# KrisKennaway/ii-vision

Measured on AMD Instinct MI355X. Metric: DHGR frames transcoded/sec, higher is better.
Workload: dtype u16; 1 GPU; DHGR NTSC palette 560x192 S-iid synthetic clips, 750 frames each, 14336 independent clips per GPU, Movie.encode control flow (490 opcodes/frame, bank flip per 2 KiB); palette=NTSC, streams_per_gpu=14336, greedy_form=shared, resident_clip_frames=750, opcodes_per_frame=490, parallelism=1 GPU x 14336 independent streams, no collective

## Files before the change

### ii-vision_amd/csrc/iiv_greedy.hip

```cpp
#include "iiv_host.h"
#include <cstdio>
#include <cstdlib>
#include <mutex>
#include <type_traits>
#include "iiv_stream.h"
#include "iiv_wave.h"

namespace iiv {

#ifndef IIV_WAVE_OCC
#define IIV_WAVE_OCC 6
#endif
#ifndef IIV_STEP_PRIO
#define IIV_STEP_PRIO 1
#endif

#ifndef IIV_SHARED_W
#define IIV_SHARED_W 8
#endif
#ifndef IIV_TAKE_CHECK_PLAIN
#define IIV_TAKE_CHECK_PLAIN 1
#endif
#ifndef IIV_TAKE_CHECK_SHARED
#define IIV_TAKE_CHECK_SHARED 0
#endif
#ifndef IIV_SHARED_W_HGR
#define IIV_SHARED_W_HGR 16
#endif
struct WaveLds {
    uint32_t nz[256];
    uint32_t pdone[256];
    uint32_t mt[624 + 256];
};
struct WaveLdsBits {
    uint32_t nz[256];
    uint32_t pdone[256];
};
#ifndef IIV_SHARED_HGR_HALVES
#define IIV_SHARED_HGR_HALVES 2
#endif
template <int MODE> struct SharedCfg {
    static constexpr int kOffsets = MODE == kDHGR ? 2 : IIV_SHARED_HGR_HALVES;
    static constexpr int kHalfBytes = 2 << (SplitTraits<MODE>::kLeftCBits + SplitTraits<MODE>::kLeftRowBits);
    static constexpr int kL1Bytes = kOffsets * kHalfBytes;
    static constexpr int kPad = kL1Bytes;
    static constexpr int kW = MODE == kDHGR ? IIV_SHARED_W : IIV_SHARED_W_HGR;
    static constexpr bool kMtRegs = MODE == kHGR && kOffsets == 2;
    static constexpr int kWaveBytes = kMtRegs ? (int)sizeof(WaveLdsBits) : (int)sizeof(WaveLds);
    static constexpr int kLds = kPad + kW * kWaveBytes;
    static_assert(kLds <= 160 * 1024, "a workgroup's LDS");
};

__device__ static inline WaveLds *own_wave_lds()
{
    __shared__ WaveLds w;
    return &w;
}

template <int MODE, int W, bool FOUR = false>
__global__ __launch_bounds__(64 * W, W == 1 ? IIV_WAVE_OCC : MODE == kHGR ? (W + 3) / 4 : (2 * W + 3) / 4 + (W % 4 ? 1 : 0)) void greedy_wave_kernel(StreamState *__restrict__ states,
                                                                   const uint8_t *__restrict__ frames_main,
                                                                   const uint8_t *__restrict__ frames_aux, int n_frames,
                                                                   const LaunchSeg *__restrict__ segs, int seg_stride,
                                                                   const NarrowTables nt,
                                                                   uint8_t *__restrict__ ops_out, size_t ops_stride, int n_streams, int bank, int *__restrict__ queue,
                                                                   int count_stats, const int *__restrict__ perm, uint32_t *__restrict__ cost)
{
    using T = SplitTraits<MODE>;
    constexpr uint32_t INF = 0xffffffffu;
    typedef uint32_t __attribute__((aligned(2))) u32_a2;
    using SC = SharedCfg<MODE>;
    extern __shared__ uint32_t dyn_lds[];
    const int lane0 = W == 1 ? (int)threadIdx.x : (int)(threadIdx.x & 63);
    const int wave = W == 1 ? 0 : IIV_SGPR(threadIdx.x >> 6);
    constexpr bool kMtRegs = W > 1 && SC::kMtRegs;
    uint32_t *nz, *pdone, *mt;
    if constexpr (W == 1) {
        __shared__ uint32_t nz_s[256], pdone_s[256], mt_s[624 + 256];
        nz = nz_s, pdone = pdone_s, mt = mt_s;
    } else if constexpr (kMtRegs) {
        WaveLdsBits *wl = reinterpret_cast<WaveLdsBits *>(reinterpret_cast<char *>(dyn_lds) + SC::kPad) + wave;
        nz = wl->nz, pdone = wl->pdone, mt = nullptr;
    } else {
        WaveLds *wl = reinterpret_cast<WaveLds *>(reinterpret_cast<char *>(dyn_lds) + SC::kPad) + wave;
        nz = wl->nz, pdone = wl->pdone, mt = wl->mt;
    }
    const char *const l1_lds = reinterpret_cast<const char *>(dyn_lds);
    if (W > 1) {
        uint4 *dst = reinterpret_cast<uint4 *>(dyn_lds);
        constexpr int kQuads = SC::kHalfBytes / 16;
#pragma unroll
        for (int h = 0; h < SC::kOffsets; h++) {
            const int o = byte_offset<MODE>(h, bank);
            const uint4 *src = reinterpret_cast<const uint4 *>(nt.base + ((size_t)o << (T::kLeftCBits + T::kLeftRowBits + 1)));
            for (int i = threadIdx.x; i < kQuads; i += 64 * W) dst[h * kQuads + i] = src[i];
        }
        __syncthreads();
    }

    auto run_stream = [&](const int stream, const int lane) {
    const unsigned long long clk0 = __builtin_amdgcn_s_memtime();
    StreamState &S = states[stream];
    const LaunchSeg g = segs[(size_t)stream * seg_stride];
    const int n_ops = IIV_SGPR(g.n_ops), is_aux = IIV_SGPR(g.is_aux), frame = IIV_SGPR(g.frame);
    if (n_ops <= 0) return;
    if (W > 1 && is_aux != bank) {
        if (lane == 0 && !S.error) S.error = kErrBankMix;
        return;
    }
    uint8_t *out = ops_out + (size_t)stream * ops_stride + (size_t)IIV_SGPR(g.ops_base) * 6;

    if (!S.gen_active || S.error) {
        if (lane == 0 && !S.error) S.error = kErrNoGenerator;
        return;
    }
    for (int i = lane; i < 256; i += 64) {
        nz[i] = S.nzbits[i];
        pdone[i] = S.pdone[i];
    }
    if constexpr (!kMtRegs)
        for (int i = lane; i < 624; i += 64) mt[i] = S.mt_py[i];
    if (W == 1) __syncthreads(); else wave_lds_sync();
    uint32_t *ahead = mt + 624;
    auto gen_ahead = [&]() {
#pragma unroll
        for (int k = 0; k < 4; k++) {
            const int i = lane + 64 * k;
            if (k < 3 || i < 227) ahead[i] = mt[i + 397] ^ mt_mix(mt[i], mt[i + 1]);
        }
        wave_lds_sync();
        {
            const int i = 192 + lane;
            if (i >= 227) ahead[i] = ahead[i - 227] ^ mt_mix(mt[i], mt[i + 1]);
        }
        wave_lds_sync();
    };
    auto gen_rest = [&]() {
#pragma unroll
        for (int k = 0; k < 6; k++) {
            const int i = 256 + 64 * k + lane;
            if (k < 5 || i < 624) {
                const uint32_t nv = i < 483 ? ahead[i - 227] : mt[i - 227];
                const uint32_t nx = i == 623 ? ahead[0] : mt[i + 1];
                const uint32_t v = nv ^ mt_mix(mt[i], nx);
                wave_lds_sync();
                mt[i] = v;
            }
            wave_lds_sync();
        }
    };
    auto move_head = [&]() {
#pragma unroll
        for (int k = 0; k < 4; k++) mt[lane + 64 * k] = ahead[lane + 64 * k];
        wave_lds_sync();
    };
    int mt_idx = IIV_SGPR(S.mt_py_idx);
    MtRegs mtr;
    const MtLaneConsts mtk(lane);
    uint32_t q_key = 0;
    int q_idx = 0, n_pend = 0, mt_behind = 0;
    constexpr int kQueueTrash = 63, kQueueHigh = 56;
    if constexpr (kMtRegs) {
        mt_regs_load(mtr, S.mt_py, lane);
        if (mt_idx >= 624) {
            mt_regs_twist(mtr, mtk);
            mt_idx -= 624;
        }
    } else {
        gen_ahead();
        if (mt_idx >= 624) {
            move_head();
            gen_rest();
            gen_ahead();
            mt_idx -= 624;
        }
    }
    bool twist_pending = false;
    auto twist_now = [&]() {
        if constexpr (!kMtRegs) {
            if (__builtin_expect(twist_pending, 0)) {
                gen_rest();
                gen_ahead();
                twist_pending = false;
            }
        }
    };

    const int n_sorted = IIV_SGPR(S.n_sorted);
    const int truncated = IIV_SGPR(S.truncated);
    int head = IIV_SGPR(S.head), n_pushed = IIV_SGPR(S.n_pushed), exhausted = IIV_SGPR(S.exhausted);
    int done = 0, err = 0;
    uint32_t draws = 0;
    unsigned long long pad_ops = 0;
    const uint32_t pad_content = (uint32_t)IIV_SGPR(S.pad_content);

    const int o_e = byte_offset<MODE>(0, is_aux), o_d = byte_offset<MODE>(1, is_aux);
    const uint32_t l1_e = (uint32_t)o_e << (T::kLeftCBits + T::kLeftRowBits + 1), l1_d = (uint32_t)o_d << (T::kLeftCBits + T::kLeftRowBits + 1);
    const uint32_t r1_e = nt.right_off + ((uint32_t)o_e << (T::kRightCBits + T::kRightRowBits + 1));
    const uint32_t r1_d = nt.right_off + ((uint32_t)o_d << (T::kRightCBits + T::kRightRowBits + 1));
    const __amdgpu_buffer_rsrc_t rsrc_s = __builtin_amdgcn_make_buffer_rsrc((void *)&S, 0, (int)sizeof(StreamState), 0x00020000);
    const int up_off = (int)offsetof(StreamState, up16) + is_aux * 8192 * 2, mem_off = (int)offsetof(StreamState, mem) + is_aux * 8192;
    const __amdgpu_buffer_rsrc_t rsrc = __builtin_amdgcn_make_buffer_rsrc((void *)nt.base, 0, 0x7fffffff, 0x00020000);
    const uint8_t *tgt_frames = (MODE == kDHGR && is_aux ? frames_aux : frames_main) +
                                ((size_t)stream * n_frames + frame) * 8192;
    const uint4 *wd_rows = reinterpret_cast<const uint4 *>(S.wd);
    const int wsel = lane >> 3;
    const int sh0 = (4 * lane) & 31;
    const uint32_t y0 = 4u * (uint32_t)lane;
    constexpr uint32_t kKeyMul = (1u << kWdDwShift) | (1u << 8);
    const uint32_t ycst0 = y0 - kNarrowBias * kKeyMul;

    struct Loaded {
        uint32_t gl[4], gr[4], kb[4];
    };
    auto gather8 = [&](const uint4 &w, uint32_t c, Loaded &L) {
        const uint32_t sl_e = (W == 1 ? l1_e : 0u) + (split_content_left<MODE>(c, 0) << (T::kLeftRowBits + 1));
        constexpr bool kOddInLds = W > 1 && SC::kOffsets == 2;
        const uint32_t sl_d = (kOddInLds ? (uint32_t)SC::kHalfBytes : l1_d) + (split_content_left<MODE>(c, 1) << (T::kLeftRowBits + 1));
        const uint32_t sr_e = r1_e + (split_content_right<MODE>(c, 0) << (T::kRightRowBits + 1));
        const uint32_t sr_d = r1_d + (split_content_right<MODE>(c, 1) << (T::kRightRowBits + 1));
        const uint32_t wr[4] = {w.x, w.y, w.z, w.w};
        uint32_t ol[4], orr[4];
#pragma unroll
        for (int r = 0; r < 4; r++) {
            ol[r] = wd_off_left(wr[r]);
            orr[r] = wd_off_right(wr[r]);
        }
        if (W == 1) {
            L.gl[0] = (uint16_t)__builtin_amdgcn_raw_buffer_load_b16(rsrc, (int)ol[0], (int)sl_e, 0);
            L.gl[2] = (uint16_t)__builtin_amdgcn_raw_buffer_load_b16(rsrc, (int)ol[2], (int)sl_e, 0);
            L.gl[1] = (uint16_t)__builtin_amdgcn_raw_buffer_load_b16(rsrc, (int)ol[1], (int)sl_d, 0);
            L.gl[3] = (uint16_t)__builtin_amdgcn_raw_buffer_load_b16(rsrc, (int)ol[3], (int)sl_d, 0);
        } else {
            L.gl[0] = *reinterpret_cast<const uint16_t *>(l1_lds + (sl_e + ol[0]));
            L.gl[2] = *reinterpret_cast<const uint16_t *>(l1_lds + (sl_e + ol[2]));
            if (kOddInLds) {
                L.gl[1] = *reinterpret_cast<const uint16_t *>(l1_lds + (sl_d + ol[1]));
                L.gl[3] = *reinterpret_cast<const uint16_t *>(l1_lds + (sl_d + ol[3]));
            } else {
                L.gl[1] = (uint16_t)__builtin_amdgcn_raw_buffer_load_b16(rsrc, (int)ol[1], (int)sl_d, 0);
                L.gl[3] = (uint16_t)__builtin_amdgcn_raw_buffer_load_b16(rsrc, (int)ol[3], (int)sl_d, 0);
            }
        }
        L.gr[0] = (uint16_t)__builtin_amdgcn_raw_buffer_load_b16(rsrc, (int)orr[0], (int)sr_e, 0);
        L.gr[2] = (uint16_t)__builtin_amdgcn_raw_buffer_load_b16(rsrc, (int)orr[2], (int)sr_e, 0);
        L.gr[1] = (uint16_t)__builtin_amdgcn_raw_buffer_load_b16(rsrc, (int)orr[1], (int)sr_d, 0);
        L.gr[3] = (uint16_t)__builtin_amdgcn_raw_buffer_load_b16(rsrc, (int)orr[3], (int)sr_d, 0);
#pragma unroll
        for (int r = 0; r < 4; r++) {
            L.kb[r] = (wr[r] << kWdDwShift) + (ycst0 + (uint32_t)r);
            asm volatile("" : "+v"(L.kb[r]));
        }
    };

    uint32_t ob0 = 0, ob1 = 0, ob2 = 0, ob3 = 0;
    int ob_base = 0, ob_n = 0;
    auto flush_ops = [&]() {
        if (lane < ob_n) {
            uint8_t *q = out + (size_t)(ob_base + lane) * 6;
            const uint32_t pg = (ob0 >> 8) & 31u, xx = ob0 & 255u, cc = (ob0 >> 16) & 255u;
            *reinterpret_cast<u32_a2 *>(q) = (pg + 32u) | (cc << 8) | (xx << 16) | (ob1 << 24);
            *reinterpret_cast<uint16_t *>(q + 4) = (uint16_t)((ob2 & 255u) | ((FOUR ? ob3 & 255u : xx) << 8));
        }
        ob_base = done;
        ob_n = 0;
    };

#ifdef IIV_STAMPS
    int n_ties = 0, n_tie_members = 0, n_ties_small = 0;
    int n_rel = 0, n_rel_single = 0, n_rel_double = 0;
#endif
    bool prev_tie = false;
    int n_exact = 0;
    uint32_t pkey_v = 0;
    int push_f1 = 0, push_f2 = 0, push_f3 = 0, push_base = 0;
    static_assert(kPushedCap >= 3 * 7680 + 8, "a generator's steps have distinct primaries: <= 7680 steps x <= 3 pushes");
    auto mt_resolve = [&](int a, int b, int off) -> uint32_t {
        const int lo = __builtin_amdgcn_readlane(q_idx, a) - off, hi = __builtin_amdgcn_readlane(q_idx, b - 1) - off;
        const bool in = lane >= a && lane < b;
        const uint32_t w = mt_regs_gather(mtr, in ? q_idx - off : lo, lo, hi);
        const uint32_t key = q_key | ((mt_temper(w) >> 24) << 13);
        const uint32_t slot = in ? (uint32_t)(n_pushed - n_pend + lane) * 4u : 0x7ffffff0u;
        __builtin_amdgcn_raw_buffer_store_b32(key, rsrc_s, (int)slot, (int)offsetof(StreamState, pushed), 0);
        return key;
    };
    auto mt_enqueue = [&](uint32_t keys, int k, int fk, int pos, int first) {
        const uint32_t key0 = (uint32_t)__builtin_amdgcn_readlane((int)keys, k);
        const int at = fk ? n_pend + pos : kQueueTrash;
        asm("s_mov_b32 m0, %4\n\tv_writelane_b32 %0, %2, m0\n\tv_writelane_b32 %1, %3, m0"
            : "+v"(q_key), "+v"(q_idx)
            : "s"(key0), "s"(first + pos), "s"(at));
    };
    auto mt_service = [&](int target) -> uint32_t {
        uint32_t keys = 0;
        for (;;) {
            const int r = (int)__popcll(__ballot(lane < n_pend && q_idx < 624));
            if (r > 0) {
                keys = mt_resolve(0, r, 0);
                if (r < n_pend) {
                    const int from = ((lane + r) & 63) << 2;
                    q_key = (uint32_t)__builtin_amdgcn_ds_bpermute(from, (int)q_key);
                    q_idx = __builtin_amdgcn_ds_bpermute(from, q_idx);
                }
                n_pend -= r;
            }
            if (mt_behind <= target) break;
            mt_regs_twist(mtr, mtk);
            mt_behind--;
            q_idx -= 624;
        }
        return keys;
    };
    auto apply = [&](auto track, uint32_t e, uint32_t W1, uint32_t W2, uint32_t W3, int C) {
        const int p = (e >> 8) & 31, x = e & 255;
        const uint32_t c = (e >> 16) & 0xffu;
        auto flag = [](uint32_t w) -> int {
            int f;
            asm("s_min_u32 %0, %1, 1" : "=s"(f) : "s"(w >> 8) : "scc");
            return f;
        };
        const int f1 = flag(W1), f2 = flag(W2), f3 = FOUR ? flag(W3) : 0;
        if (__builtin_expect(n_pushed > kPushedCap - 4, 0)) {
            err = kErrPushedOverflow;
            return;
        }
        if (__builtin_expect(twist_pending && mt_idx + C + (FOUR ? 3 : 2) >= 256, 0)) twist_now();
        uint32_t w_v = (uint32_t)x, k_v = 0u;
        asm("v_writelane_b32 %0, %2, 1\n\tv_writelane_b32 %0, %3, 2\n\tv_writelane_b32 %1, %4, 2"
            : "+v"(w_v), "+v"(k_v)
            : "s"(W1), "s"(W2), "s"(f1));
        if (FOUR)
            asm("v_writelane_b32 %0, %2, 3\n\tv_writelane_b32 %1, %3, 3" : "+v"(w_v), "+v"(k_v) : "s"(W3), "s"(f1 + f2));
        asm("s_mov_b32 m0, %4\n\tv_writelane_b32 %0, %3, m0\n\tv_writelane_b32 %1, %5, m0\n\tv_writelane_b32 %2, %6, m0"
            : "+v"(ob0), "+v"(ob1), "+v"(ob2)
            : "s"(IIV_SGPR(e)), "s"(ob_n), "s"(W1), "s"(W2));
        if (FOUR) asm("s_mov_b32 m0, %2\n\tv_writelane_b32 %0, %1, m0" : "+v"(ob3) : "s"(W3), "s"(ob_n));
        int ln = lane;
        asm volatile("" : "+v"(ln));
        uint32_t pk0_v = 0;
        if (ln < (FOUR ? 4 : 3)) {
            const uint32_t off = w_v & 255u, val = w_v >> 8;
            const uint32_t loc = (uint32_t)(p * 256) | off;
            __builtin_amdgcn_raw_buffer_store_b16((unsigned short)val, rsrc_s, (int)(loc * 2u), up_off, 0);
            __builtin_amdgcn_raw_buffer_store_b8((unsigned char)c, rsrc_s, (int)loc, mem_off, 0);
            const uint32_t gone_bit = (val == 0u ? 1u : 0u) << (off & 31u);
            atomicAnd(&nz[loc >> 5], ~gone_bit);
            atomicOr(&pdone[p * 8 + (x >> 5)], 1u << (x & 31));
            if constexpr (!kMtRegs) {
                const uint32_t nonce = mt_temper(mt[mt_idx + C + (int)k_v]) >> 24;
                const uint32_t pkey = ((2047u - val) << 21) | (nonce << 13) | loc;
                const uint32_t slot = val != 0u ? (uint32_t)(n_pushed + (int)k_v) * 4u : 0x7ffffff0u;
                __builtin_amdgcn_raw_buffer_store_b32(pkey, rsrc_s, (int)slot, (int)offsetof(StreamState, pushed), 0);
                if (decltype(track)::value) pkey_v = pkey;
            } else {
                pk0_v = ((2047u - val) << 21) | loc;
            }
        }
        if constexpr (kMtRegs) {
            const int first = mt_behind * 624 + mt_idx + C;
            mt_enqueue(pk0_v, 1, f1, 0, first);
            mt_enqueue(pk0_v, 2, f2, f1, first);
            if (FOUR) mt_enqueue(pk0_v, 3, f3, f1 + f2, first);
            n_pend += f1 + f2 + f3;
        }
        if (decltype(track)::value) push_f1 = f1, push_f2 = f2, push_f3 = f3, push_base = n_pushed;
        mt_idx += C + f1 + f2 + f3;
        draws += (uint32_t)(C + f1 + f2 + f3);
        n_pushed += f1 + f2 + f3;
        if constexpr (kMtRegs) {
            if (decltype(track)::value) {
                pkey_v = mt_service(0);
                if (n_pend > 0) {
                    const int r = (FOUR ? f1 + f2 + f3 : f1 + f2) - n_pend;
                    const uint32_t k2 = (uint32_t)__builtin_amdgcn_ds_bpermute(((lane - r) & 63) << 2, (int)mt_service(-1));
                    pkey_v = lane < r ? pkey_v : k2;
                }
            } else if (__builtin_expect(n_pend > kQueueHigh, 0)) {
                (void)mt_service(0);
            }
        }
        done++;
        ob_n++;
        if (__builtin_expect(ob_n == 64, 0)) flush_ops();
        if (__builtin_expect(mt_idx >= 624, 0)) {
            if constexpr (kMtRegs) {
                mt_idx -= 624;
                mt_behind++;
            } else {
                move_head();
                mt_idx -= 624;
                twist_pending = true;
            }
        }
    };

    auto step = [&](auto track, uint32_t e, const Loaded &L, uint32_t nzw, uint32_t pdw) -> bool {
        const int x = e & 255;
        const uint32_t c = (e >> 16) & 0xffu;
        const uint32_t xword = (uint32_t)__builtin_amdgcn_readlane((int)nzw, (x >> 5) * 8);
        if (__builtin_expect(!((xword >> (x & 31)) & 1u), 0)) return false;
        if (MODE == kDHGR && c >= 0x80) {
            err = kErrPaletteBit;
            return true;
        }
        const uint32_t xbit = wsel == (x >> 5) ? 1u << (x & 31) : 0u;
        nzw &= ~xbit;
        pdw |= xbit;
        uint32_t nd[4];
        int ke[4];
        int C = 0;
        unsigned long long cand[4];
#pragma unroll
        for (int r = 0; r < 4; r++) {
            nd[r] = L.gl[r] + L.gr[r];
            const int d = (int)(__umul24(nd[r], kKeyMul) + L.kb[r]);
            const int gone = __builtin_amdgcn_sbfe((int)pdw, sh0 + r, 1);
            const int live = __builtin_amdgcn_sbfe((int)nzw, sh0 + r, 1);
            ke[r] = d & live;
            cand[r] = __ballot((d & ~gone) < 0);
            C += (int)__popcll(cand[r]);
        }
        const int a0 = ke[0] < ke[1] ? ke[0] : ke[1], b0 = ke[0] < ke[1] ? ke[1] : ke[0];
        const int a1 = ke[2] < ke[3] ? ke[2] : ke[3], b1 = ke[2] < ke[3] ? ke[3] : ke[2];
        const int k1 = a0 < a1 ? a0 : a1, hi01 = a0 < a1 ? a1 : a0, mb = b0 < b1 ? b0 : b1;
        const int k2 = hi01 < mb ? hi01 : mb;
        const int k3 = hi01 < mb ? mb : hi01;
        auto nd_of = [&](int y) -> uint32_t {
            const uint32_t nd01 = nd[0] | (nd[1] << 16), nd23 = nd[2] | (nd[3] << 16);
            const uint32_t pa = (uint32_t)__builtin_amdgcn_readlane((int)nd01, y >> 2);
            const uint32_t pb = (uint32_t)__builtin_amdgcn_readlane((int)nd23, y >> 2);
            return ((((y & 2) ? pb : pa) >> ((y & 1) * 16)) & 0xffffu) - kNarrowBias;
        };
        uint32_t W1 = (uint32_t)x, W2 = (uint32_t)x, W3 = (uint32_t)x;
        bool tie = prev_tie;
        auto shared_delta = [&](int K) -> bool {
            uint32_t m = ((uint32_t)(ke[0] ^ K)) - 1u;
#pragma unroll
            for (int r = 1; r < 4; r++) {
                const uint32_t x1 = ((uint32_t)(ke[r] ^ K)) - 1u;
                m = x1 < m ? x1 : m;
            }
            return __ballot(m < (1u << kWdDwShift) - 1u) != 0ull;
        };
#ifdef IIV_STAMPS
        {
            int D1 = k1, D2 = k2;
            wave_top2_i32(D1, D2);
            if (D1 < 0 && D2 < 0 && ((D1 >> kWdDwShift) == (D2 >> kWdDwShift) || shared_delta(D2))) {
                int n1 = 0;
#pragma unroll
                for (int r = 0; r < 4; r++) n1 += (int)__popcll(__ballot(ke[r] < 0 && (ke[r] >> kWdDwShift) == (D1 >> kWdDwShift)));
                n_ties++;
                n_tie_members += n1;
                if (n1 <= 2) n_ties_small++;
                const int dR = n1 >= 2 ? (D1 >> kWdDwShift) : (D2 >> kWdDwShift);
                int lane_cnt = 0;
#pragma unroll
                for (int r = 0; r < 4; r++) lane_cnt += (ke[r] < 0 && (ke[r] >> kWdDwShift) == dR) ? 1 : 0;
                const unsigned long long b1 = __ballot(lane_cnt >= 1), b2 = __ballot(lane_cnt >= 2), b3 = __ballot(lane_cnt >= 3), b4 = __ballot(lane_cnt >= 4);
                n_rel += IIV_SGPR(__popcll(b1) + __popcll(b2) + __popcll(b3) + __popcll(b4));
                n_rel_single += IIV_SGPR(b2 == 0ull ? 1 : 0);
                n_rel_double += IIV_SGPR((b2 != 0ull && b3 == 0ull) ? 1 : 0);
            }
        }
#endif
        int K1 = k1, K2 = k2;
        if (!tie) wave_top2_i32(K1, K2); else K1 = K2 = 0;
        if (__builtin_expect(K1 < 0, 1)) {
            W1 = (uint32_t)K1 & 0x7ffffu;
            if (__builtin_expect(K2 < 0, 1)) {
                W2 = (uint32_t)K2 & 0x7ffffu;
                tie = (K1 >> kWdDwShift) == (K2 >> kWdDwShift);
                if constexpr (!FOUR) {
                    if (!tie) tie = shared_delta(K2);
                } else if (!tie) {
                    const int c3 = k1 > K2 ? k1 : (k2 > K2 ? k2 : k3);
                    const int K3 = wave_min_i32(c3);
                    if (K3 < 0) {
                        W3 = (uint32_t)K3 & 0x7ffffu;
                        tie = (K2 >> kWdDwShift) == (K3 >> kWdDwShift) || shared_delta(K3);
                    }
                }
            }
        }
        if (W > 1 ? __builtin_expect(tie, 0) : tie) {
            twist_now();
            n_exact++;
            static_assert(kWdDwShift == 20, "the key's delta field is taken from bits 20..31 of an eligible key");
            int key[4];
            int run = mt_idx;
#pragma unroll
            for (int q = 0; q < 4; q++) run += prefix_popc(cand[q]);
            uint32_t word[4];
            if constexpr (kMtRegs) {
                int at[4];
                bool mine[4];
#pragma unroll
                for (int r = 0; r < 4; r++) {
                    at[r] = run;
                    mine[r] = (cand[r] >> lane) & 1ull;
                    run += mine[r] ? 1 : 0;
                }
                const int last = mt_idx + (C > 0 ? C - 1 : 0), last0 = last < 623 ? last : 623;
                if (mt_behind != 0) (void)mt_service(0);
#pragma unroll
                for (int r = 0; r < 4; r++) word[r] = mt_regs_gather(mtr, mine[r] && at[r] < 624 ? at[r] : mt_idx, mt_idx, last0);
                if (__builtin_expect(last >= 624, 0)) {
                    (void)mt_service(-1);
#pragma unroll
                    for (int r = 0; r < 4; r++) {
                        const uint32_t w2 = mt_regs_gather(mtr, mine[r] && at[r] >= 624 ? at[r] - 624 : 0, 0, last - 624);
                        word[r] = at[r] >= 624 ? w2 : word[r];
                    }
                }
            } else {
#pragma unroll
                for (int r = 0; r < 4; r++) {
                    word[r] = mt[run];
                    run += (int)((cand[r] >> lane) & 1ull);
                }
            }
#pragma unroll
            for (int r = 0; r < 4; r++) {
                const uint32_t nonce = mt_temper(word[r]) >> 24;
                key[r] = (int)(((uint32_t)(ke[r] >> 4) & 0xffff0000u) | (nonce << 8) | (y0 + r));
            }
            const int ta0 = key[0] < key[1] ? key[0] : key[1], tb0 = key[0] < key[1] ? key[1] : key[0];
            const int ta1 = key[2] < key[3] ? key[2] : key[3], tb1 = key[2] < key[3] ? key[3] : key[2];
            const int t1 = ta0 < ta1 ? ta0 : ta1;
            const int thi = ta0 < ta1 ? ta1 : ta0, tmb = tb0 < tb1 ? tb0 : tb1;
            const int t2 = thi < tmb ? thi : tmb;
            int T1 = t1, T2 = t2;
            wave_top2_i32(T1, T2);
            W1 = T1 < 0 ? (nd_of(T1 & 255) << 8) | (uint32_t)(T1 & 255) : (uint32_t)x;
            W2 = T2 < 0 ? (nd_of(T2 & 255) << 8) | (uint32_t)(T2 & 255) : (uint32_t)x;
            prev_tie = T2 < 0 && (T1 >> 16) == (T2 >> 16);
            if constexpr (FOUR) {
                const int t3 = thi < tmb ? tmb : thi;
                const int T3 = wave_min_i32(t1 > T2 ? t1 : (t2 > T2 ? t2 : t3));
                W3 = T3 < 0 ? (nd_of(T3 & 255) << 8) | (uint32_t)(T3 & 255) : (uint32_t)x;
                prev_tie = prev_tie || (T3 < 0 && (T2 >> 16) == (T3 >> 16));
            }
        }
        apply(track, e, W1, W2, W3, C);
        return true;
    };

    int guard = n_ops + 8192 + 2 * kPushedCap + 64;
#ifdef IIV_STAMPS
    unsigned long long ph[4] = {0, 0, 0, 0}, ph_t = __builtin_amdgcn_s_memtime();
    const unsigned long long wave_t0 = ph_t, wave_r0 = __builtin_amdgcn_s_memrealtime();
    int n_steps = 0;
#define IIV_PHASE(i)                                                  \
    do {                                                              \
        const unsigned long long now_ = __builtin_amdgcn_s_memtime(); \
        ph[i] += now_ - ph_t;                                         \
        ph_t = now_;                                                  \
    } while (0)
#else
#define IIV_PHASE(i) do { } while (0)
#endif

    if (head < n_sorted && !exhausted) {
        int win_base = head, win_end = head;
        int n_dense = 0, qi = 0;
        uint32_t dense_e = 0;
        uint32_t ord_next = S.order[(head + lane) & 8191];
        auto refill = [&]() {
            const int start = win_end;
            const uint32_t e = ord_next;
            const int idx = start + lane;
            ord_next = S.order[(idx + 64) & 8191];
            const uint32_t loc = e & 0x1fffu;
            const bool v = idx < n_sorted && ((nz[loc >> 5] >> (loc & 31)) & 1u);
            const unsigned long long mask = __ballot(v);
            n_dense = (int)__popcll(mask);
            qi = 0;
            const int dst = v ? prefix_popc(mask) : n_dense + prefix_popc(~mask);
            dense_e = (uint32_t)__builtin_amdgcn_ds_permute(dst << 2, (int)((e & 0x00ffffffu) | ((uint32_t)lane << 24)));
            asm volatile("" : "+v"(dense_e));
            win_base = start;
            win_end = start + 64 < n_sorted ? start + 64 : n_sorted;
        };
        auto take = [&](int &next_head) -> uint32_t {
            for (;;) {
                while (__builtin_expect(qi >= n_dense, 0)) {
                    if (win_end >= n_sorted) return 0u;
                    refill();
                }
                const uint32_t e = (uint32_t)__builtin_amdgcn_readlane((int)dense_e, qi++);
                if constexpr ((W == 1 && IIV_TAKE_CHECK_PLAIN) || (W > 1 && IIV_TAKE_CHECK_SHARED)) {
                    const uint32_t loc = e & 0x1fffu;
                    const uint32_t w = IIV_SGPR(nz[loc >> 5]);
                    if (!((w >> (loc & 31)) & 1u)) continue;
                }
                next_head = win_base + (int)(e >> 24) + 1;
                return e | 0x80000000u;
            }
        };
        auto row_of = [&](uint32_t e) -> uint4 { return wd_rows[((e >> 8) & 31) * 64 + lane]; };

        uint32_t eA, eB, eC;
        int hA = head, hB, hC;
        uint4 rowP, rowQ;
        Loaded set0, set1;
        eA = take(hA);
        const uint4 rowA = row_of(eA);
        hB = hA;
        eB = eA ? take(hB) : 0u;
        rowP = row_of(eB);
        gather8(rowA, eA >> 16 & 0xffu, set0);
        hC = hB;
        eC = eB ? take(hC) : 0u;
        rowQ = row_of(eC);
        auto half = [&](const Loaded &cur, Loaded &nxt, uint4 &row, bool active) -> bool {
#ifdef IIV_STAMPS
            asm volatile("" : "+v"(row.x), "+v"(row.y), "+v"(row.z), "+v"(row.w));
            IIV_PHASE(3);
#endif
            const uint32_t nzA = nz[((eA >> 8) & 31) * 8 + wsel], pdA = pdone[((eA >> 8) & 31) * 8 + wsel];
            gather8(row, eB >> 16 & 0xffu, nxt);
            __builtin_amdgcn_sched_barrier(0);
            int hD = hC;
            const uint32_t eD = (active && eC) ? take(hD) : 0u;
            row = row_of(eD);
            IIV_PHASE(0);
            if (__builtin_expect(!active, 0)) return false;
            twist_now();
            IIV_PHASE(1);
#ifdef IIV_STAMPS
            n_steps++;
#endif
            __builtin_amdgcn_s_setprio(IIV_STEP_PRIO);
            (void)step(std::false_type{}, eA, cur, nzA, pdA);
            __builtin_amdgcn_s_setprio(0);
            IIV_PHASE(2);
            head = hA;
            eA = eB;
            hA = hB;
            eB = eC;
            hB = hC;
            eC = eD;
            hC = hD;
            if (__builtin_expect(--guard < 0, 0)) err = kErrGuard;
            return eA && done < n_ops && !err;
        };
        if (eA && done < n_ops) {
            bool more;
            do {
                more = half(set0, set1, rowP, true);
                more = half(set1, set0, rowQ, more);
            } while (more);
        }
        if (!eA && !err) head = n_sorted;
    }

    if (done < n_ops && !err && !exhausted) {
        if constexpr (kMtRegs) (void)mt_service(0);
        uint32_t ck = INF, ci = 0;
        for (int i = lane; i < n_pushed; i += 64) {
            const uint32_t k = S.pushed[i];
            ci = k < ck ? (uint32_t)i : ci;
            ck = k < ck ? k : ck;
        }
        auto writelane = [&](uint32_t &v, uint32_t val, int l) {
            asm("s_mov_b32 m0, %2\n\tv_writelane_b32 %0, %1, m0" : "+v"(v) : "s"(IIV_SGPR(val)), "s"(IIV_SGPR(l)));
        };
        auto wave_min_u32 = [&](uint32_t v) -> uint32_t { return (uint32_t)wave_min_i32((int)(v ^ 0x80000000u)) ^ 0x80000000u; };
        auto cache_merge = [&](uint32_t key, uint32_t idx) {
            const int sub = (int)(idx & 63u);
            const uint32_t cur = (uint32_t)__builtin_amdgcn_readlane((int)ck, sub);
            if (key < cur) {
                writelane(ck, key, sub);
                writelane(ci, idx, sub);
            }
        };
        while (done < n_ops && !err) {
            if (--guard < 0) {
                err = kErrGuard;
                break;
            }
            if (truncated) {
                err = kErrSortBudget;
                break;
            }
            const uint32_t bk = wave_min_u32(ck);
            if (bk == INF) {
                exhausted = 1;
                break;
            }
            const int wl = (int)__builtin_ctzll(__ballot(ck == bk));
            const uint32_t bi = (uint32_t)__builtin_amdgcn_readlane((int)ci, wl);
            if (lane == 0) S.pushed[bi] = INF;
            constexpr int kSub = (kPushedCap + 4095) / 4096;
            static_assert(kPushedCap <= 64 * 64 * kSub, "the rescan of a sub-bag must reach every index below kPushedCap");
            uint32_t rk[kSub], ridx[kSub];
#pragma unroll
            for (int t = 0; t < kSub; t++) {
                ridx[t] = (uint32_t)wl + 64u * (uint32_t)(lane + 64 * t);
                rk[t] = INF;
                if (ridx[t] < (uint32_t)n_pushed && ridx[t] != bi) rk[t] = S.pushed[ridx[t]];
            }
            const uint32_t loc = bk & 0x1fffu;
            const uint32_t c = (uint32_t)IIV_SGPR(tgt_frames[loc]);
            const uint32_t e = loc | (c << 16);
            const uint4 w = wd_rows[((e >> 8) & 31) * 64 + lane];
            Loaded L;
            gather8(w, c, L);
            twist_now();
            push_f1 = push_f2 = push_f3 = 0;
            (void)step(std::true_type{}, e, L, nz[((e >> 8) & 31) * 8 + wsel], pdone[((e >> 8) & 31) * 8 + wsel]);
            uint32_t mk = rk[0], mi = ridx[0];
#pragma unroll
            for (int t = 1; t < kSub; t++) {
                mi = rk[t] < mk ? ridx[t] : mi;
                mk = rk[t] < mk ? rk[t] : mk;
            }
            const uint32_t nk = wave_min_u32(mk);
            const uint32_t ni = (uint32_t)__builtin_amdgcn_readlane((int)mi, (int)__builtin_ctzll(__ballot(mk == nk)));
            writelane(ck, nk, wl);
            writelane(ci, ni, wl);
            if (push_f1) cache_merge((uint32_t)__builtin_amdgcn_readlane((int)pkey_v, kMtRegs ? 0 : 1), (uint32_t)push_base);
            if (push_f2) cache_merge((uint32_t)__builtin_amdgcn_readlane((int)pkey_v, kMtRegs ? push_f1 : 2), (uint32_t)(push_base + push_f1));
            if (FOUR && push_f3) cache_merge((uint32_t)__builtin_amdgcn_readlane((int)pkey_v, kMtRegs ? push_f1 + push_f2 : 3), (uint32_t)(push_base + push_f1 + push_f2));
        }
    }

    flush_ops();
    if (exhausted && done < n_ops && !err) {
        for (int i = done + lane; i < n_ops; i += 64) {
            uint8_t *q = out + (size_t)i * 6;
            q[0] = 32; q[1] = (uint8_t)pad_content; q[2] = 0; q[3] = 0; q[4] = 0; q[5] = 0;
        }
        pad_ops += (unsigned long long)(n_ops - done);
        done = n_ops;
    }
    twist_now();
    if constexpr (kMtRegs) (void)mt_service(0);
    if (W == 1) __syncthreads(); else wave_lds_sync();
    for (int i = lane; i < 256; i += 64) {
        S.nzbits[i] = nz[i];
        S.pdone[i] = pdone[i];
    }
    if constexpr (kMtRegs) mt_regs_store(mtr, S.mt_py, lane);
    else
        for (int i = lane; i < 624; i += 64) S.mt_py[i] = mt[i];
    if (lane == 0) {
        S.mt_py_idx = mt_idx;
        S.head = head;
        S.n_pushed = n_pushed;
        S.exhausted = exhausted;
        if (exhausted) S.out_of_work[is_aux] = 1;
        S.draws_py += (unsigned long long)draws;
        S.ops += (unsigned long long)done;
        S.pad_ops += pad_ops;
        if (err && S.error == 0) S.error = err;
        if (cost) cost[stream] = (uint32_t)(__builtin_amdgcn_s_memtime() - clk0);
        if (count_stats) {
            S.stat_exact += (unsigned long long)n_exact;
            S.stat_ops += (unsigned long long)(done - (int)pad_ops);
            S.stat_runs += 1ull;
        }
#ifdef IIV_STAMPS
        for (int i = 0; i < 4; i++) S.stamps[16 + i] = ph[i];
        S.stamps[24] = wave_t0;
        S.stamps[25] = __builtin_amdgcn_s_memtime();
        S.stamps[26] = (unsigned long long)done;
        S.stamps[27] = (unsigned long long)n_steps;
        S.stamps[29] = wave_r0;
        S.stamps[30] = __builtin_amdgcn_s_memrealtime();
        S.stamps[31] = (unsigned long long)n_ties | ((unsigned long long)n_ties_small << 20) | ((unsigned long long)n_tie_members << 40);
        S.stamps[20] = (unsigned long long)n_rel;
        S.stamps[21] = (unsigned long long)n_rel_single | ((unsigned long long)n_rel_double << 32);
        S.stamps[28] = ((unsigned long long)__builtin_amdgcn_s_getreg((20 ) | (0 << 6) | (31 << 11)) << 32) |
                       (unsigned)__builtin_amdgcn_s_getreg((4 ) | (0 << 6) | (31 << 11));
#endif
    }
    };

    if constexpr (W == 1) {
        run_stream(perm ? IIV_SGPR(perm[blockIdx.x]) : (int)blockIdx.x, lane0);
    } else {
        for (;;) {
            int next = 0;
            if (lane0 == 0) next = atomicAdd(queue, 1);
            next = IIV_SGPR(next);
            if (next >= n_streams) break;
            if (perm) next = IIV_SGPR(perm[next]);
            int lane_i = lane0;
            asm volatile("" : "+v"(lane_i));
            run_stream(next, lane_i);
            wave_lds_sync();
        }
    }
}
#undef IIV_PHASE

template <int MODE, bool FOUR> static int launch_shared(const GreedyArgs &a, hipStream_t st)
{
    using SC = SharedCfg<MODE>;
    constexpr int kMaxDev = 64;
    static int resident_of[kMaxDev] = {};
    static std::mutex mu;
    int dev = 0;
    if (hip_check(hipGetDevice(&dev), "hipGetDevice")) return IIV_ERR_HIP;
    if (dev < 0 || dev >= kMaxDev) return set_error(IIV_ERR_INVALID, "greedy_wave_kernel: device index %d", dev);
    int resident;
    {
        std::lock_guard<std::mutex> lock(mu);
        if (!resident_of[dev]) {
            int per_cu = 0;
            hipDeviceProp_t prop;
            if (hip_check(hipFuncSetAttribute((const void *)greedy_wave_kernel<MODE, SC::kW, FOUR>, hipFuncAttributeMaxDynamicSharedMemorySize, SC::kLds),
                          "greedy_wave_kernel LDS attribute") ||
                hip_check(hipOccupancyMaxActiveBlocksPerMultiprocessor(&per_cu, (const void *)greedy_wave_kernel<MODE, SC::kW, FOUR>, 64 * SC::kW, (size_t)SC::kLds),
                          "greedy_wave_kernel occupancy") ||
                hip_check(hipGetDeviceProperties(&prop, dev), "hipGetDeviceProperties"))
                return IIV_ERR_HIP;
            resident_of[dev] = (per_cu > 0 ? per_cu : 1) * prop.multiProcessorCount;
        }
        resident = resident_of[dev];
    }
    const int wgs = (a.n_streams + SC::kW - 1) / SC::kW;
    hipLaunchKernelGGL((greedy_wave_kernel<MODE, SC::kW, FOUR>), dim3(wgs < resident ? wgs : resident), dim3(64 * SC::kW), (size_t)SC::kLds, st, a.states,
                       a.frames_main, a.frames_aux, a.n_frames, a.segs, a.seg_stride, a.nt, a.ops_out, a.ops_stride, a.n_streams, a.uniform_bank, a.queue, a.count_stats ? 1 : 0, a.perm, a.cost);
    return IIV_OK;
}

int launch_greedy_wave(int mode, const GreedyArgs &a, hipStream_t st, int *form_out)
{
    const bool shared = a.shared && a.uniform_bank >= 0 && a.queue && a.lds_pad == 0;
    if (form_out) *form_out = shared ? 1 : 0;
    int rc = IIV_OK;
    if (shared && a.fourth)
        rc = mode == kDHGR ? launch_shared<kDHGR, true>(a, st) : launch_shared<kHGR, true>(a, st);
    else if (a.fourth && mode == kDHGR)
        hipLaunchKernelGGL((greedy_wave_kernel<kDHGR, 1, true>), dim3(a.n_streams), dim3(64), (size_t)a.lds_pad, st, a.states, a.frames_main,
                           a.frames_aux, a.n_frames, a.segs, a.seg_stride, a.nt, a.ops_out, a.ops_stride, a.n_streams, a.uniform_bank, (int *)nullptr, a.count_stats ? 1 : 0, a.perm, a.cost);
    else if (a.fourth)
        hipLaunchKernelGGL((greedy_wave_kernel<kHGR, 1, true>), dim3(a.n_streams), dim3(64), (size_t)a.lds_pad, st, a.states, a.frames_main,
                           a.frames_aux, a.n_frames, a.segs, a.seg_stride, a.nt, a.ops_out, a.ops_stride, a.n_streams, a.uniform_bank, (int *)nullptr, a.count_stats ? 1 : 0, a.perm, a.cost);
    else if (shared)
        rc = mode == kDHGR ? launch_shared<kDHGR, false>(a, st) : launch_shared<kHGR, false>(a, st);
    else if (mode == kDHGR)
        hipLaunchKernelGGL((greedy_wave_kernel<kDHGR, 1>), dim3(a.n_streams), dim3(64), (size_t)a.lds_pad, st, a.states, a.frames_main,
                           a.frames_aux, a.n_frames, a.segs, a.seg_stride, a.nt, a.ops_out, a.ops_stride, a.n_streams, a.uniform_bank, (int *)nullptr, a.count_stats ? 1 : 0, a.perm, a.cost);
    else
        hipLaunchKernelGGL((greedy_wave_kernel<kHGR, 1>), dim3(a.n_streams), dim3(64), (size_t)a.lds_pad, st, a.states, a.frames_main,
                           a.frames_aux, a.n_frames, a.segs, a.seg_stride, a.nt, a.ops_out, a.ops_stride, a.n_streams, a.uniform_bank, (int *)nullptr, a.count_stats ? 1 : 0, a.perm, a.cost);
    if (rc) return rc;
    return hip_check(hipGetLastError(), "greedy_wave_kernel launch");
}

}
```

Baseline: 3.548 million frames/s.

## Batch MT twist LDS passes, prefetch nonce words early, load rows via buffer loads

For shared-wave mode, the Mersenne Twister regeneration now reads each lane's source words into registers first and writes them back in two passes, instead of syncing around every 64-word chunk, which cuts the number of wave LDS barriers. Nonce MT words are read from LDS before the top-2 reduction, so their latency overlaps with that work rather than sitting inside apply. Row fetches switch to raw 128-bit buffer loads addressed from the stream state descriptor. Stamp instrumentation is extended with more phases. The two-pass twist relies on an ordering argument about overlapping reads and writes of the state, so a mistake there would silently corrupt the random sequence.

```diff
diff --git a/ii-vision_amd/csrc/iiv_greedy.hip b/ii-vision_amd/csrc/iiv_greedy.hip
--- a/ii-vision_amd/csrc/iiv_greedy.hip
+++ b/ii-vision_amd/csrc/iiv_greedy.hip
@@ -26,6 +26,15 @@
 #endif
 #ifndef IIV_SHARED_W_HGR
 #define IIV_SHARED_W_HGR 16
+#endif
+#ifndef IIV_MT_TWO_TRIPS
+#define IIV_MT_TWO_TRIPS 1
+#endif
+#ifndef IIV_NONCE_EARLY
+#define IIV_NONCE_EARLY 1
+#endif
+#ifndef IIV_ROW_BUFFER_LOAD
+#define IIV_ROW_BUFFER_LOAD 1
 #endif
 struct WaveLds {
     uint32_t nz[256];
@@ -136,6 +145,31 @@
         wave_lds_sync();
     };
     auto gen_rest = [&]() {
+      if constexpr (W > 1 && IIV_MT_TWO_TRIPS) {
+        uint32_t own[6], nxt[6], far[6];
+#pragma unroll
+        for (int k = 0; k < 6; k++) {
+            const int i = 256 + 64 * k + lane;
+            own[k] = mt[i];
+            nxt[k] = mt[i + 1];
+            if (k < 3) far[k] = ahead[i - 227];
+        }
+        wave_lds_sync();
+#pragma unroll
+        for (int k = 0; k < 3; k++) mt[256 + 64 * k + lane] = far[k] ^ mt_mix(own[k], nxt[k]);
+        wave_lds_sync();
+#pragma unroll
+        for (int k = 3; k < 6; k++) {
+            const int i = 256 + 64 * k + lane;
+            far[k] = (k == 3 && i < 483) ? ahead[i - 227] : mt[i - 227];
+        }
+#pragma unroll
+        for (int k = 3; k < 6; k++) {
+            const int i = 256 + 64 * k + lane;
+            if (k < 5 || i < 624) mt[i] = far[k] ^ mt_mix(own[k], nxt[k]);
+        }
+        wave_lds_sync();
+      } else {
 #pragma unroll
         for (int k = 0; k < 6; k++) {
             const int i = 256 + 64 * k + lane;
@@ -148,6 +182,7 @@
             }
             wave_lds_sync();
         }
+      }
     };
     auto move_head = [&]() {
 #pragma unroll
@@ -311,7 +346,20 @@
         }
         return keys;
     };
-    auto apply = [&](auto track, uint32_t e, uint32_t W1, uint32_t W2, uint32_t W3, int C) {
+#ifdef IIV_STAMPS
+    unsigned long long ph[7] = {0, 0, 0, 0, 0, 0, 0}, ph_t = __builtin_amdgcn_s_memtime();
+    const unsigned long long wave_t0 = ph_t, wave_r0 = __builtin_amdgcn_s_memrealtime();
+    int n_steps = 0;
+#define IIV_PHASE(i)                                                  \
+    do {                                                              \
+        const unsigned long long now_ = __builtin_amdgcn_s_memtime(); \
+        ph[i] += now_ - ph_t;                                         \
+        ph_t = now_;                                                  \
+    } while (0)
+#else
+#define IIV_PHASE(i) do { } while (0)
+#endif
+    auto apply = [&](auto track, uint32_t e, uint32_t W1, uint32_t W2, uint32_t W3, int C, const uint32_t (&nw)[3]) {
         const int p = (e >> 8) & 31, x = e & 255;
         const uint32_t c = (e >> 16) & 0xffu;
         auto flag = [](uint32_t w) -> int {
@@ -347,7 +395,12 @@
             atomicAnd(&nz[loc >> 5], ~gone_bit);
             atomicOr(&pdone[p * 8 + (x >> 5)], 1u << (x & 31));
             if constexpr (!kMtRegs) {
-                const uint32_t nonce = mt_temper(mt[mt_idx + C + (int)k_v]) >> 24;
+#if IIV_NONCE_EARLY
+                const uint32_t nword = FOUR ? (k_v == 0u ? nw[0] : k_v == 1u ? nw[1] : nw[2]) : (k_v == 0u ? nw[0] : nw[1]);
+#else
+                const uint32_t nword = mt[mt_idx + C + (int)k_v];
+#endif
+                const uint32_t nonce = mt_temper(nword) >> 24;
                 const uint32_t pkey = ((2047u - val) << 21) | (nonce << 13) | loc;
                 const uint32_t slot = val != 0u ? (uint32_t)(n_pushed + (int)k_v) * 4u : 0x7ffffff0u;
                 __builtin_amdgcn_raw_buffer_store_b32(pkey, rsrc_s, (int)slot, (int)offsetof(StreamState, pushed), 0);
@@ -413,6 +466,13 @@
 #pragma unroll
         for (int r = 0; r < 4; r++) {
             nd[r] = L.gl[r] + L.gr[r];
+#ifdef IIV_STAMPS
+            if (r == 0) {
+                uint32_t s1 = L.gl[1] + L.gr[1], s2 = L.gl[2] + L.gr[2], s3 = L.gl[3] + L.gr[3];
+                asm volatile("" : "+v"(nd[0]), "+v"(s1), "+v"(s2), "+v"(s3));
+                IIV_PHASE(4);
+            }
+#endif
             const int d = (int)(__umul24(nd[r], kKeyMul) + L.kb[r]);
             const int gone = __builtin_amdgcn_sbfe((int)pdw, sh0 + r, 1);
             const int live = __builtin_amdgcn_sbfe((int)nzw, sh0 + r, 1);
@@ -464,6 +524,16 @@
             }
         }
 #endif
+        uint32_t nw[3] = {0u, 0u, 0u};
+#if IIV_NONCE_EARLY
+        if constexpr (!kMtRegs) {
+            if (__builtin_expect(twist_pending && mt_idx + C + (FOUR ? 3 : 2) >= 256, 0)) twist_now();
+            nw[0] = mt[mt_idx + C];
+            nw[1] = mt[mt_idx + C + 1];
+            if (FOUR) nw[2] = mt[mt_idx + C + 2];
+        }
+#endif
+        IIV_PHASE(5);
         int K1 = k1, K2 = k2;
         if (!tie) wave_top2_i32(K1, K2); else K1 = K2 = 0;
         if (__builtin_expect(K1 < 0, 1)) {
@@ -542,25 +612,12 @@
                 prev_tie = prev_tie || (T3 < 0 && (T2 >> 16) == (T3 >> 16));
             }
         }
-        apply(track, e, W1, W2, W3, C);
+        IIV_PHASE(6);
+        apply(track, e, W1, W2, W3, C, nw);
         return true;
     };
 
     int guard = n_ops + 8192 + 2 * kPushedCap + 64;
-#ifdef IIV_STAMPS
-    unsigned long long ph[4] = {0, 0, 0, 0}, ph_t = __builtin_amdgcn_s_memtime();
-    const unsigned long long wave_t0 = ph_t, wave_r0 = __builtin_amdgcn_s_memrealtime();
-    int n_steps = 0;
-#define IIV_PHASE(i)                                                  \
-    do {                                                              \
-        const unsigned long long now_ = __builtin_amdgcn_s_memtime(); \
-        ph[i] += now_ - ph_t;                                         \
-        ph_t = now_;                                                  \
-    } while (0)
-#else
-#define IIV_PHASE(i) do { } while (0)
-#endif
-
     if (head < n_sorted && !exhausted) {
         int win_base = head, win_end = head;
         int n_dense = 0, qi = 0;
@@ -598,7 +655,16 @@
                 return e | 0x80000000u;
             }
         };
+#if IIV_ROW_BUFFER_LOAD
+        typedef uint32_t u32x4 __attribute__((ext_vector_type(4)));
+        const int row_lane_off = lane * 16;
+        auto row_of = [&](uint32_t e) -> uint4 {
+            const u32x4 r = __builtin_amdgcn_raw_buffer_load_b128(rsrc_s, row_lane_off, (int)offsetof(StreamState, wd) + (int)((e >> 8) & 31) * 1024, 0);
+            return make_uint4(r.x, r.y, r.z, r.w);
+        };
+#else
         auto row_of = [&](uint32_t e) -> uint4 { return wd_rows[((e >> 8) & 31) * 64 + lane]; };
+#endif
 
         uint32_t eA, eB, eC;
         int hA = head, hB, hC;
@@ -763,10 +829,12 @@
         }
 #ifdef IIV_STAMPS
         for (int i = 0; i < 4; i++) S.stamps[16 + i] = ph[i];
+        S.stamps[22] = ph[4];
+        S.stamps[23] = ph[5];
         S.stamps[24] = wave_t0;
         S.stamps[25] = __builtin_amdgcn_s_memtime();
         S.stamps[26] = (unsigned long long)done;
-        S.stamps[27] = (unsigned long long)n_steps;
+        S.stamps[27] = (unsigned long long)n_steps | (ph[6] << 32);
         S.stamps[29] = wave_r0;
         S.stamps[30] = __builtin_amdgcn_s_memrealtime();
         S.stamps[31] = (unsigned long long)n_ties | ((unsigned long long)n_ties_small << 20) | ((unsigned long long)n_tie_members << 40);
```

Measured after the change: 3.575 million frames/s (median of 6 runs). About the same (+0.8%).
